# lijrjyan/SDVAR

Measured on AMD Instinct MI355X. Metric: images/s (+ mean accepted tokens/step), VAR-d16 256^2 B=8, d12 draft + d16 verify, per GPU, higher is better.
Workload: dtype f32 (GEMM operands split into 2 fp16 planes to 2^-22, 3 fp16 MFMA products, fp32 accumulate); 1 GPU; BASELINE.json P1: VAR-d16 256^2 B=8/GPU, d12 draft + d16 verify, gamma=2, cfg=1.5 top_k=900 top_p=0.96, acceptance=natural, incl. VQVAE decode (overlapped with the next batch on a 2nd stream); verifier one round behind the draft once gamma = 1; parallelism=1 independent batch shards

## Files before the change

### sdvar_amd/csrc/api.hip

```cpp
#include <math.h>
#include <stdarg.h>
#include <string.h>

#include <vector>

#include "../../include/sdvar_hip.h"
#include "common.h"
#include <string>

namespace sdvar {

int gemm_f32_nt(const float* X, int ldx, const float* W, const float* bias, float* out, int ldo, int M, int N, int K, int epi,
                const float* res, int ldres, const float* gate, int rows_per_gate, int gate_stride, hipStream_t stream);
struct PendingSplitK { const float* ws; const float* bias; const float* gate; int split, rows_per_gate, gate_stride; };
int ln_modulate(float* x, const float* scale, const float* shift, float* out, uint16_t* outp, size_t ops, int rows, int C, int rows_per_img, int mod_stride, const PendingSplitK* pend, int pfmt, hipStream_t stream);
float* splitk_workspace(size_t* floats);
float* set_splitk_workspace(float* p);
size_t splitk_workspace_floats();
int qk_norm_append(const float* qkv, const float* scale_mul, float* q_out, void* k_cache, void* v_cache, int kv_f16, int R, int l, int H, int Lmax, int pos0, const PendingSplitK* pend, int v_only, hipStream_t stream);
int gemm_f16x2_qkv(const uint16_t* X, size_t xps, const uint16_t* W, size_t wps, const float* wsi, const float* bias, float* out, int ldo, int M, int N, int K,
                   const float* scale_mul, float* q_out, void* k_cache, void* v_cache, int l, int H, int Lp, int pos0, int kv_fmt, int* defer, int* fused, hipStream_t stream);
bool gemm_f16x2_rowblk_ok(int M, int N, int K, int ln, int qkv);
bool gemm_f16x2_rowblk_want(int M, int C, int V, int rows_per_img);
int gemm_f16x2_rowblk(const float* x, int ldx, const float* scale, const float* shift, int rows_per_img, int mod_stride, const uint16_t* X, size_t xps,
// ... 9 lines not shown
int build_lvl_pos(const float* lvl_embed, const float* pos, const int* stage_of_tok, float* out, int L, int C, hipStream_t stream);
int embed_next(const float* nxt, const float* Ww, const float* bw, const float* lvl_pos, float* x, int B, int l, int C, int t0, int ltot, int tok_off, int pair, hipStream_t stream);
int xent_stats(const float* logits, const long long* targets, int B, int L, int V, int tail, float* nll_out, long long* argmax_out, double* sums, int accumulate,
               hipStream_t stream);
int attention_f32(const float* q, const void* kc, const void* vc, int kv_f16, float* out, uint16_t* outp, size_t ops, int pfmt, int R, int H, int l, int Lmax, int Ktot, int n_chunk, const int* qbeg, const int* vis, hipStream_t stream);
int gemm_bf16x3_nt(const uint16_t* X, size_t xps, const uint16_t* W, size_t wps, const float* bias, float* out, int ldo, uint16_t* outp, size_t ops,
                   int M, int N, int K, int epi, const float* res, int ldres, const float* gate, int rows_per_gate, int gate_stride, int* defer, hipStream_t stream);
int attention_masked(const float* q, const void* kc, const void* vc, int fmt, const float* bias, float* out, uint16_t* outp, size_t ops, int pfmt, int R, int H, int l,
                     int Lmax, int Ktot, hipStream_t stream);
int split_planes(const float* x, uint16_t* planes, int rows, int cols, size_t plane_stride, hipStream_t stream);
int gemm_f16x2_nt(const uint16_t* X, size_t xps, const uint16_t* W, size_t wps, const float* wsi, const float* bias, float* out, int ldo, uint16_t* outp, size_t ops,
                  int M, int N, int K, int epi, const float* res, int ldres, const float* gate, int rows_per_gate, int gate_stride, int* defer, hipStream_t stream);
int split_planes_f16(const float* x, uint16_t* planes, int rows, int cols, size_t plane_stride, const float* scale, hipStream_t stream);
int weight_scale_f16(const float* w, size_t n, float* sc, hipStream_t stream);
void debug_set_gemm_cfg_h(int bm, int split);
void debug_set_gemm_cfg_p(int bm, int split);
void debug_set_gemm_stamps(unsigned long long* p);
void debug_set_qkv_fuse(int on);
void debug_set_h4_var(int v);
void debug_set_h2_stages(int v);
void debug_set_small_pp(int v);
void debug_set_attn_pp_sched(int v);
void debug_set_conv_pp(int v);
void debug_get_gemm_cfg_h(int* out);
int planes_guard(const uint16_t* h_plane, size_t n, unsigned long long* cnt, hipStream_t stream);
int cfg_sample(const float* logits, int B, int l, int V, float one_plus_t, float t, int top_k, int use_top_p, float top_p_thr, const float* q, uint64_t seed,
               uint32_t draw, uint32_t image_offset, long long* ids, int ids_stride, float* dbg_masked, hipStream_t stream);
int noise_fill(float* q, int B, int l, int V, uint64_t seed, uint32_t draw, uint32_t image_offset, hipStream_t stream);
int verify_accept(const float* logits, int B, int lsum, int V, int n_chunk, const int* qbeg, const float* one_plus_t, const float* t, const long long* draft_ids,
                  int ids_stride, double thr, int mode, int top_k, float kl_thr, const float* draft_logits, const long long* dl_off, int* counts,
                  long long* argmax_out, unsigned char* match_out, long long* corrected_out, hipStream_t stream);
int cfg_combine(const float* logits, int B, int lsum, int V, int n_chunk, const int* qbeg, const float* one_plus_t, const float* t, float* out, hipStream_t stream);
int gumbel_mix(const float* masked, int B, int l, int V, float scale, float tau, const float* e, uint64_t seed, uint32_t draw, uint32_t image_offset,
               const float* codebook, int Cv, float* h, hipStream_t stream);
void debug_set_gemm_cfg(int bm, int split);
int quant_code_norms(const float* codebook, float* e2, int V, int Cv, hipStream_t stream);
int quant_nearest(const float* z, int N, int P, const float* codebook, const float* e2, int V, int Cv, long long* ids, int ids_stride, hipStream_t stream);
int quant_encode_stage(float* f_rest, float* f_hat, float* z, float* up_scratch, const float* codebook, const float* e2, const float* Wdn_si, const float* Wup_si,
                       const float* phi_w, const float* phi_b, long long* ids, int ids_stride, int B, int pn, int HW, int V, int Cv, int last, hipStream_t stream);
int quant_next(const long long* ids, int ids_stride, const float* hvec, const float* codebook, const float* Wup, const float* phi_w, const float* phi_b, const float* Wdn,
               float* up_scratch, const float* f_in, float* f_hat, float* nxt, int B, int pn, int pn_next, int HW, int Cv, int last, hipStream_t stream);

enum { EPI_BIAS = 0, EPI_BIAS_GELU = 1, EPI_GATED_RES = 2 };

static thread_local char g_err[1024] = "";
void set_error(const char* fmt, ...) {
// ... 786 lines not shown
    return SDVAR_OK;
}

int sdvar_debug_set_qkv_fuse(int32_t on) { debug_set_qkv_fuse(on); return SDVAR_OK; }
int sdvar_debug_set_rowblk(int32_t on) { debug_set_rowblk(on); return SDVAR_OK; }
int sdvar_op_gemm_rowblk(const float* x, int32_t ldx, const float* scale, const float* shift, int32_t rows_per_img, int32_t mod_stride, const uint16_t* Xp, uint64_t x_plane_stride,
                         const uint16_t* Wp, uint64_t w_plane_stride, const float* w_scale, const float* bias, float* out, int32_t ldo, uint16_t* out_planes, uint64_t out_plane_stride,
                         int32_t M, int32_t N, int32_t K, int32_t epi, const float* res, int32_t ldres, const float* gate, int32_t rows_per_gate, int32_t gate_stride,
                         const float* scale_mul, float* q_out, void* k_cache, void* v_cache, int32_t l, int32_t H, int32_t Lp, int32_t pos0, int32_t kv_fmt, void* stream) {
    SDVAR_CHECK_ARG(gemm_f16x2_rowblk_ok(M, N, K, x != nullptr, q_out != nullptr), "op_gemm_rowblk: M=%d N=%d K=%d outside the row-block kernel's range (M <= 80; K <= 1024 with a LayerNorm operand, <= 4096 with planes) or the kernel is switched off", M, N, K);
    ProfScope ps(9, 2.0 * M * N * K, 4.0 * ((double)M * K + (double)N * K + (double)M * N), (hipStream_t)stream);
    return gemm_f16x2_rowblk(x, ldx, scale, shift, rows_per_img, mod_stride, Xp, (size_t)x_plane_stride, Wp, (size_t)w_plane_stride, w_scale ? w_scale + 1 : nullptr, bias, out, ldo, out_planes,
                             (size_t)out_plane_stride, M, N, K, epi, res, ldres, gate, rows_per_gate, gate_stride, scale_mul, q_out, k_cache, v_cache, l, H, Lp, pos0, kv_fmt, (hipStream_t)stream);
}

int sdvar_debug_set_variant(const char* name, int32_t value) {
    SDVAR_CHECK_ARG(name, "debug_set_variant: null name");
    const std::string n(name);
    if (n == "gemm_h4_var") { SDVAR_CHECK_ARG(value <= 3, "gemm_h4_var %d", value); debug_set_h4_var(value); }
    else if (n == "gemm_h2_stages") { SDVAR_CHECK_ARG(value < 0 || value == 2 || value == 3 || value == 4 || value == 5 || value == 6, "gemm_h2_stages %d", value); debug_set_h2_stages(value); }
    else if (n == "gemm_small_pp") { SDVAR_CHECK_ARG(value <= 2, "gemm_small_pp %d", value); debug_set_small_pp(value); }
    else if (n == "attn_pp_sched") { SDVAR_CHECK_ARG(value <= 3, "attn_pp_sched %d", value); debug_set_attn_pp_sched(value); }
    else if (n == "conv_pp") { SDVAR_CHECK_ARG(value <= 2, "conv_pp %d", value); debug_set_conv_pp(value); }
    else { set_error("debug_set_variant: unknown variant '%s'", name); return SDVAR_ERR_ARG; }
    return SDVAR_OK;
}

int sdvar_debug_get_gemm_cfg(int32_t* out4) {
    SDVAR_CHECK_ARG(out4, "debug_get_gemm_cfg: null");
    int v[4]; debug_get_gemm_cfg_h(v);
    for (int i = 0; i < 4; ++i) out4[i] = v[i];
    return SDVAR_OK;
}

int sdvar_debug_set_f16x2_guard(int32_t on) {
    if (on && !g_guard_cnt) {
        SDVAR_HIP(hipMalloc((void**)&g_guard_cnt, 4 * sizeof(unsigned long long)));
        SDVAR_HIP(hipMemset(g_guard_cnt, 0, 4 * sizeof(unsigned long long)));
    }
    g_guard_on = on != 0;
    return SDVAR_OK;
}

int sdvar_debug_get_f16x2_guard(uint64_t* out4, int32_t reset) {
    SDVAR_CHECK_ARG(out4, "debug_get_f16x2_guard: null");
    for (int i = 0; i < 4; ++i) out4[i] = 0;
// ... 35 lines not shown
```

### sdvar_amd/csrc/conv.hip

```cpp
#include <stdlib.h>

#include "common.h"

#ifdef SDVAR_TIMING_EXPERIMENTS
#define SDVAR_CDBG(a, bit) ((a).dbg & (bit))
#else
#define SDVAR_CDBG(a, bit) 0
#endif

namespace sdvar {
static int g_conv_pp_override = -1;
void debug_set_conv_pp(int v) { g_conv_pp_override = v; }


typedef __bf16 bf16x8 __attribute__((ext_vector_type(8)));
typedef _Float16 f16x8 __attribute__((ext_vector_type(8)));
typedef __attribute__((address_space(3))) void* lds_ptr_t;
typedef const __attribute__((address_space(1))) void* glb_ptr_t;

enum { CEPI_BIAS = 0, CEPI_BIAS_RES = 1, CEPI_PARTIAL = 2 };
constexpr int CBM = 256, CBN = 160;
constexpr int CSTAGE = 3 * (CBM + CBN) * 32;
constexpr int CSTAGE_H = 2 * (CBM + CBN) * 32;

struct ConvArgs {
    const uint16_t* X; const uint16_t* W;
    size_t xps, wps;
    size_t x_rows;
    int x_row0;
    const float* wsi;
    const float* bias; const float* res; float* out;
    int M, N, cb, taps, ih, iw, ldo, split, k_per_split;
    double* gn_part; int cpg;
    int up_phase;
    size_t w_phase_stride;
    int dbg;
};

template <int EPI>
__device__ __forceinline__ void conv_epilogue(const ConvArgs& a, f32x16 (&acc)[5], float wsi, int m0, int n0, int tm, int ks, int phase, int wave, int li, int lh,
                                              int tid, uint16_t* csm) {
    float rv[5][16];
    if (EPI == CEPI_BIAS_RES) {
#pragma unroll
        for (int j = 0; j < 5; ++j) {
            const int n = n0 + j * 32 + li;
#pragma unroll
            for (int r = 0; r < 16; ++r) {
                const int m = m0 + wave * 32 + (r & 3) + 8 * (r >> 2) + 4 * lh;
                rv[j][r] = (n < a.N && m < a.M) ? a.res[(size_t)m * a.ldo + n] : 0.f;
            }
        }
    }
#pragma unroll
    for (int j = 0; j < 5; ++j) {
        const int n = n0 + j * 32 + li;
        if (n >= a.N) continue;
        const float bv = (EPI != CEPI_PARTIAL && a.bias) ? a.bias[n] : 0.f;
        float* outp = (EPI == CEPI_PARTIAL) ? a.out + (size_t)ks * a.M * a.ldo : a.out;
#pragma unroll
// ... 30 lines not shown
        }
        __syncthreads();
        const int gl = tid, col0 = gl * a.cpg;
        if (col0 < CBN && n0 + col0 < a.N) {
            double a1 = 0.0, a2 = 0.0;
            for (int w = 0; w < 8; ++w)
                for (int c = 0; c < a.cpg; ++c) { a1 += (double)red[w * 160 + col0 + c]; a2 += (double)red[1280 + w * 160 + col0 + c]; }
            double* o = a.gn_part + ((size_t)(a.up_phase >= 0 ? 4 * tm + phase : tm) * 32 + (n0 + col0) / a.cpg) * 2;
            o[0] = a1; o[1] = a2;
        }
    }
}

typedef float cf32x4 __attribute__((ext_vector_type(4)));
__device__ __forceinline__ float dpp_row_sum16(float v) {
    v += __builtin_bit_cast(float, __builtin_amdgcn_update_dpp(0, __builtin_bit_cast(int, v), 0x111, 0xF, 0xF, true));
    v += __builtin_bit_cast(float, __builtin_amdgcn_update_dpp(0, __builtin_bit_cast(int, v), 0x112, 0xF, 0xF, true));
    v += __builtin_bit_cast(float, __builtin_amdgcn_update_dpp(0, __builtin_bit_cast(int, v), 0x114, 0xF, 0xF, true));
    v += __builtin_bit_cast(float, __builtin_amdgcn_update_dpp(0, __builtin_bit_cast(int, v), 0x118, 0xF, 0xF, true));
    return v;
}
template <int EPI>
__device__ __forceinline__ void conv_epilogue16(const ConvArgs& a, cf32x4 (&acc)[2][10], float wsi, int m0, int n0, int tm, int ks, int phase, int wave, int l15, int lq,
                                                int tid, uint16_t* csm) {
    int mrow[2]; size_t orow[2];
#pragma unroll
    for (int mt = 0; mt < 2; ++mt) {
        const int m = m0 + wave * 32 + 16 * mt + l15;
        mrow[mt] = m; orow[mt] = (size_t)m;
        if (EPI != CEPI_PARTIAL && a.up_phase >= 0 && m < a.M) {
            const int hw = a.ih * a.iw, b = m / hw, rem = m - b * hw, y = rem / a.iw, x = rem - y * a.iw;
            orow[mt] = ((size_t)(b * 2 * a.ih + 2 * y + (phase >> 1)) * (2 * a.iw) + 2 * x + (phase & 1));
        }
    }
    cf32x4 rv[2][10];
    if (EPI == CEPI_BIAS_RES) {
#pragma unroll
        for (int mt = 0; mt < 2; ++mt)
#pragma unroll
            for (int nt = 0; nt < 10; ++nt) {
                const int n = n0 + 16 * nt + 4 * lq;
                rv[mt][nt] = (n < a.N && mrow[mt] < a.M) ? *reinterpret_cast<const cf32x4*>(a.res + (size_t)mrow[mt] * a.ldo + n) : cf32x4{0.f, 0.f, 0.f, 0.f};
            }
    }
    float* outp = (EPI == CEPI_PARTIAL) ? a.out + (size_t)ks * a.M * a.ldo : a.out;
#pragma unroll
    for (int nt = 0; nt < 10; ++nt) {
        const int n = n0 + 16 * nt + 4 * lq;
        if (n >= a.N) continue;
        const cf32x4 bv = (EPI != CEPI_PARTIAL && a.bias) ? *reinterpret_cast<const cf32x4*>(a.bias + n) : cf32x4{0.f, 0.f, 0.f, 0.f};
#pragma unroll
        for (int mt = 0; mt < 2; ++mt) {
            if (mrow[mt] >= a.M) continue;
            cf32x4 v;
#pragma unroll
            for (int e = 0; e < 4; ++e) { v[e] = acc[mt][nt][e] * wsi + bv[e]; if (EPI == CEPI_BIAS_RES) v[e] += rv[mt][nt][e]; }
            if (!SDVAR_CDBG(a, 4)) *reinterpret_cast<cf32x4*>(outp + orow[mt] * a.ldo + n) = v;
            acc[mt][nt] = v;
        }
    }
    if (EPI != CEPI_PARTIAL && a.gn_part && !SDVAR_CDBG(a, 2)) {
        float* red = reinterpret_cast<float*>(csm);
        __syncthreads();
#pragma unroll
        for (int nt = 0; nt < 10; ++nt)
#pragma unroll
            for (int e = 0; e < 4; ++e) {
                const bool in = n0 + 16 * nt + 4 * lq < a.N;
                const float x0 = in ? acc[0][nt][e] : 0.f, x1 = in ? acc[1][nt][e] : 0.f;
                const float s1 = dpp_row_sum16(x0 + x1), s2 = dpp_row_sum16(x0 * x0 + x1 * x1);
                if (l15 == 15) { red[wave * 160 + 16 * nt + 4 * lq + e] = s1; red[1280 + wave * 160 + 16 * nt + 4 * lq + e] = s2; }
            }
        __syncthreads();
        const int gl = tid, col0 = gl * a.cpg;
        if (col0 < CBN && n0 + col0 < a.N) {
            double a1 = 0.0, a2 = 0.0;
            for (int w = 0; w < 8; ++w)
                for (int c = 0; c < a.cpg; ++c) { a1 += (double)red[w * 160 + col0 + c]; a2 += (double)red[1280 + w * 160 + col0 + c]; }
            double* o = a.gn_part + ((size_t)(a.up_phase >= 0 ? 4 * tm + phase : tm) * 32 + (n0 + col0) / a.cpg) * 2;
            o[0] = a1; o[1] = a2;
        }
    }
}

template <int EPI>
// ... 94 lines not shown
                __builtin_amdgcn_sched_barrier(0);
                if (s == 0 && j == 0) {
                    SDVAR_LDS_RD(fb[1][1][4], ab1, 18432);
                    SDVAR_RD_B(1, ab1, 0, 0);
                }
                if (pf) {
                    const int grp = 5 * s + j;
                    issue_one(nst, grp);
                    if (grp >= 8) issue_one(nst, grp + 2);
                }
                __builtin_amdgcn_sched_barrier(0);
            }
        }
#undef SDVAR_RD_B
#undef SDVAR_LDS_RD
    }

    conv_epilogue<EPI>(a, acc, 1.0f, m0, n0, tm, ks, phase, wave, li, lh, tid, csm);
}

template <int EPI, int PP>
__global__ __launch_bounds__(512, 2) void conv_f16x2_kernel(ConvArgs a) {
    extern __shared__ __attribute__((aligned(16))) uint16_t csm[];
    const int tiles_m = (a.M + CBM - 1) / CBM, tiles_n = (a.N + CBN - 1) / CBN, ntile = tiles_m * tiles_n;
    const int ks = blockIdx.x / ntile;
    const int lid = xcd_remap(blockIdx.x - ks * ntile, ntile);
    const int tm = lid / tiles_n, tn = lid - tm * tiles_n;
    const int m0 = tm * CBM, n0 = tn * CBN;

    const int tid = threadIdx.x, lane = tid & 63, wave = tid >> 6;
    const int li = lane & 31, lh = lane >> 5;
    const int phase = a.up_phase >= 0 ? (int)blockIdx.y : 0;
    const uint16_t* Wp = a.W + (size_t)phase * a.w_phase_stride;

    const int r16 = lane >> 2;
    const int xr0 = 32 * wave + r16, xr1 = xr0 + 16, wr0 = 16 * wave + r16, wr1 = 128 + wr0;
    const int cx0 = (lane & 3) ^ ((xr0 >> 2) & 3), cx1 = (lane & 3) ^ ((xr1 >> 2) & 3), cw0 = (lane & 3) ^ ((wr0 >> 2) & 3), cw1 = (lane & 3) ^ ((wr1 >> 2) & 3);
    const int nkt = a.taps * a.cb;
    const int kt0 = ks * a.k_per_split;
    const int nk = min(nkt - kt0, a.k_per_split);
    const int w2 = a.iw + 2;
    auto prow = [&](int m) {
        const int hw = a.ih * a.iw, b = m / hw, rem = m - b * hw, y = rem / a.iw, x = rem - y * a.iw;
        return (size_t)(b * (a.ih + 2) + y + 1) * w2 + x + 1;
    };
    const int swave = __builtin_amdgcn_readfirstlane(wave);
    const uint32_t lx0 = (uint32_t)((a.x_row0 + prow(min(m0 + xr0, a.M - 1))) * 32 + 8 * cx0) * 2u;
    const uint32_t lx1 = (uint32_t)((a.x_row0 + prow(min(m0 + xr1, a.M - 1))) * 32 + 8 * cx1) * 2u;
    const uint32_t lw0 = (uint32_t)(min(n0 + wr0, a.N - 1) * 32 + 8 * cw0) * 2u, lw1 = (uint32_t)(min(n0 + wr1, a.N - 1) * 32 + 8 * cw1) * 2u;
    const bool two_w = swave < 2;
    const char* ux = nullptr; const char* uw = nullptr;
    const int tw = (a.taps == 9) ? 3 : 2;
    int sc = kt0 % a.cb, stap = kt0 / a.cb, sty = stap / tw, stx = stap - sty * tw, skb = kt0;
    auto set_next = [&]() {
        const int shift = (a.taps == 9) ? (sty - 1) * w2 + (stx - 1) : (a.taps == 4) ? (sty - 1 + (phase >> 1)) * w2 + (stx - 1 + (phase & 1)) : 0;
        ux = reinterpret_cast<const char*>(a.X) + ((long long)sc * (long long)a.x_rows + shift) * 64;
        uw = reinterpret_cast<const char*>(Wp) + (size_t)skb * a.N * 64;
        ++skb;
        if (++sc == a.cb) { sc = 0; if (++stx == tw) { stx = 0; ++sty; } }
    };
    auto issue_one = [&](uint16_t* st, int q) {
        if (q < 6) {
            const int p = q / 3, kind = q % 3;
            if (kind == 0) SDVAR_DMA16(lx0, ux + p * a.xps * 2, SDVAR_LDS_ADDR(st + p * 8192 + swave * 1024));
            else if (kind == 1) SDVAR_DMA16(lx1, ux + p * a.xps * 2, SDVAR_LDS_ADDR(st + p * 8192 + swave * 1024 + 512));
            else SDVAR_DMA16(lw0, uw + p * a.wps * 2, SDVAR_LDS_ADDR(st + 2 * 8192 + p * 5120 + swave * 512));
        } else if (two_w) {
            const int p = q - 6;
            SDVAR_DMA16(lw1, uw + p * a.wps * 2, SDVAR_LDS_ADDR(st + 2 * 8192 + p * 5120 + 4096 + swave * 512));
        }
    };

    f32x16 acc[5];
#pragma unroll
    for (int j = 0; j < 5; ++j)
#pragma unroll
        for (int r = 0; r < 16; ++r) acc[j][r] = 0.f;

    const int sw = (li >> 2) & 3;
    const int offa = (wave * 32 + li) * 32, offb = 2 * 8192 + li * 32;
    const int ch0 = 8 * ((0 + lh) ^ sw), ch1 = 8 * ((2 + lh) ^ sw);

    set_next();
#pragma unroll
    for (int q = 0; q < 8; ++q) issue_one(csm, q);
    if (nk > 1) {
        set_next();
#pragma unroll
        for (int q = 0; q < 8; ++q) issue_one(csm + CSTAGE_H, q);
    }
    if constexpr (PP == 2) {
        const int late = __builtin_amdgcn_readfirstlane(wave >> 2);
        const int l15 = lane & 15, lq = lane >> 4;
        auto wait_next = [&](int t) {
            if (t + 2 < nk) { if (two_w) asm volatile("s_waitcnt vmcnt(8)" ::: "memory"); else asm volatile("s_waitcnt vmcnt(6)" ::: "memory"); }
            else asm volatile("s_waitcnt vmcnt(0)" ::: "memory");
        };
#define SDVAR_C_SLOT() do { __builtin_amdgcn_sched_barrier(0); __builtin_amdgcn_s_barrier(); __builtin_amdgcn_sched_barrier(0); } while (0)
#define SDVAR_LDS_RD(dst, addr, off) asm volatile("ds_read_b128 %0, %1 offset:" #off : "=v"(dst) : "v"(addr) : "memory")
#define SDVAR_C_MFMA16(J0)                                                                                      \
        _Pragma("unroll") for (int j = 0; j < 5; ++j)                                                           \
            _Pragma("unroll") for (int i = 0; i < 2; ++i) {                                                     \
                acc16[i][(J0) + j] = __builtin_amdgcn_mfma_f32_16x16x32_f16(fw[j][0], fx[i][1], acc16[i][(J0) + j], 0, 0, 0);   \
                acc16[i][(J0) + j] = __builtin_amdgcn_mfma_f32_16x16x32_f16(fw[j][1], fx[i][0], acc16[i][(J0) + j], 0, 0, 0);   \
                acc16[i][(J0) + j] = __builtin_amdgcn_mfma_f32_16x16x32_f16(fw[j][0], fx[i][0], acc16[i][(J0) + j], 0, 0, 0);   \
            }
        cf32x4 acc16[2][10];
#pragma unroll
        for (int i = 0; i < 2; ++i)
#pragma unroll
            for (int j = 0; j < 10; ++j)
#pragma unroll
                for (int r = 0; r < 4; ++r) acc16[i][j][r] = 0.f;
        const uint32_t fro = (uint32_t)(l15 * 64 + 16 * (lq ^ ((l15 >> 2) & 3)));
        const uint32_t fxo = (uint32_t)(wave * 32 * 64) + fro, fwo = 32768u + fro;
        wait_next(-1);
        SDVAR_C_SLOT();
        if (late) SDVAR_C_SLOT();
        f16x8 fx[2][2], fw[5][2];
#pragma unroll 1
        for (int t = 0; t < nk; ++t) {
            const bool pf = t + 2 < nk;
            uint16_t* nst = csm + ((t + 2) % 3) * CSTAGE_H;
            const uint32_t sb = (uint32_t)(uintptr_t)(lds_ptr_t)(csm + (t % 3) * CSTAGE_H);
            const uint32_t xa = sb + fxo, wa = sb + fwo;
            SDVAR_LDS_RD(fx[0][0], xa, 0); SDVAR_LDS_RD(fx[0][1], xa, 16384); SDVAR_LDS_RD(fx[1][0], xa, 1024); SDVAR_LDS_RD(fx[1][1], xa, 17408);
            SDVAR_LDS_RD(fw[0][0], wa, 0);    SDVAR_LDS_RD(fw[0][1], wa, 10240); SDVAR_LDS_RD(fw[1][0], wa, 1024); SDVAR_LDS_RD(fw[1][1], wa, 11264);
            SDVAR_LDS_RD(fw[2][0], wa, 2048); SDVAR_LDS_RD(fw[2][1], wa, 12288); SDVAR_LDS_RD(fw[3][0], wa, 3072); SDVAR_LDS_RD(fw[3][1], wa, 13312);
            SDVAR_LDS_RD(fw[4][0], wa, 4096); SDVAR_LDS_RD(fw[4][1], wa, 14336);
            if (pf) {
                set_next();
#pragma unroll
                for (int q = 0; q < 4; ++q) issue_one(nst, q);
            }
            asm volatile("s_waitcnt lgkmcnt(0)" ::: "memory");
            SDVAR_C_SLOT();
            SDVAR_C_MFMA16(0);
            SDVAR_C_SLOT();
            SDVAR_LDS_RD(fw[0][0], wa, 5120); SDVAR_LDS_RD(fw[0][1], wa, 15360); SDVAR_LDS_RD(fw[1][0], wa, 6144); SDVAR_LDS_RD(fw[1][1], wa, 16384);
            SDVAR_LDS_RD(fw[2][0], wa, 7168); SDVAR_LDS_RD(fw[2][1], wa, 17408); SDVAR_LDS_RD(fw[3][0], wa, 8192); SDVAR_LDS_RD(fw[3][1], wa, 18432);
            SDVAR_LDS_RD(fw[4][0], wa, 9216); SDVAR_LDS_RD(fw[4][1], wa, 19456);
            if (pf) {
#pragma unroll
                for (int q = 4; q < 8; ++q) issue_one(nst, q);
            }
            if (late) wait_next(t);
            asm volatile("s_waitcnt lgkmcnt(0)" ::: "memory");
            SDVAR_C_SLOT();
            SDVAR_C_MFMA16(5);
            if (!late) wait_next(t);
            SDVAR_C_SLOT();
        }
        if (!late) SDVAR_C_SLOT();
#undef SDVAR_C_MFMA16
#undef SDVAR_LDS_RD
#undef SDVAR_C_SLOT
        if (SDVAR_CDBG(a, 1)) return;
        conv_epilogue16<EPI>(a, acc16, a.wsi ? *a.wsi : 1.0f, m0, n0, tm, ks, phase, wave, l15, lq, tid, csm);
        return;
    } else
    if (PP) {
        const int late = __builtin_amdgcn_readfirstlane(wave >> 2);
        auto wait_next = [&](int t) {
            if (t + 2 < nk) { if (two_w) asm volatile("s_waitcnt vmcnt(8)" ::: "memory"); else asm volatile("s_waitcnt vmcnt(6)" ::: "memory"); }
            else asm volatile("s_waitcnt vmcnt(0)" ::: "memory");
        };
#define SDVAR_C_SLOT() do { __builtin_amdgcn_sched_barrier(0); __builtin_amdgcn_s_barrier(); __builtin_amdgcn_sched_barrier(0); } while (0)
#define SDVAR_LDS_RD(dst, addr, off) asm volatile("ds_read_b128 %0, %1 offset:" #off : "=v"(dst) : "v"(addr) : "memory")
#define SDVAR_RD_B(ab, p, pb) SDVAR_LDS_RD(fb[p][0], ab, pb); SDVAR_LDS_RD(fb[p][1], ab, pb + 2048); SDVAR_LDS_RD(fb[p][2], ab, pb + 4096); \
                              SDVAR_LDS_RD(fb[p][3], ab, pb + 6144); SDVAR_LDS_RD(fb[p][4], ab, pb + 8192)
#define SDVAR_C_MFMA()                                                                                  \
        _Pragma("unroll") for (int j = 0; j < 5; ++j) {                                                 \
            acc[j] = __builtin_amdgcn_mfma_f32_32x32x16_f16(fa[1], fb[0][j], acc[j], 0, 0, 0);          \
            acc[j] = __builtin_amdgcn_mfma_f32_32x32x16_f16(fa[0], fb[1][j], acc[j], 0, 0, 0);          \
            acc[j] = __builtin_amdgcn_mfma_f32_32x32x16_f16(fa[0], fb[0][j], acc[j], 0, 0, 0);          \
        }
        wait_next(-1);
        SDVAR_C_SLOT();
        if (late) SDVAR_C_SLOT();
        f16x8 fa[2], fb[2][5];
#pragma unroll 1
// ... 52 lines not shown
#undef SDVAR_RD_B
#undef SDVAR_LDS_RD
#pragma unroll
        for (int s = 0; s < 2; ++s) {
            if (s == 0) asm volatile("s_waitcnt lgkmcnt(12)" ::: "memory");
            else asm volatile("s_waitcnt lgkmcnt(0)" ::: "memory");
            __builtin_amdgcn_sched_barrier(0);
#pragma unroll
            for (int j = 0; j < 5; ++j) {
                acc[j] = __builtin_amdgcn_mfma_f32_32x32x16_f16(fa[s][1], fb[s][0][j], acc[j], 0, 0, 0);
                acc[j] = __builtin_amdgcn_mfma_f32_32x32x16_f16(fa[s][0], fb[s][1][j], acc[j], 0, 0, 0);
                acc[j] = __builtin_amdgcn_mfma_f32_32x32x16_f16(fa[s][0], fb[s][0][j], acc[j], 0, 0, 0);
                __builtin_amdgcn_sched_barrier(0);
                if (pf) {
                    const int grp = 5 * s + j;
                    if (grp < 8) issue_one(nst, grp);
                }
                __builtin_amdgcn_sched_barrier(0);
            }
        }
    }
    if (SDVAR_CDBG(a, 1)) return;
    conv_epilogue<EPI>(a, acc, a.wsi ? *a.wsi : 1.0f, m0, n0, tm, ks, phase, wave, li, lh, tid, csm);
}

__global__ __launch_bounds__(256) void conv_reduce_kernel(const float* __restrict__ ws, int split, const float* __restrict__ bias, const float* res,
                                                          float* out, int M, int N) {
    const int nv = N >> 2;
    const size_t total = (size_t)M * nv, slab = (size_t)M * N;
    for (size_t i = (size_t)blockIdx.x * blockDim.x + threadIdx.x; i < total; i += (size_t)gridDim.x * blockDim.x) {
        const int n = (int)(i % nv) * 4;
        f32x4 acc = *reinterpret_cast<const f32x4*>(ws + 4 * i);
        for (int s = 1; s < split; ++s) {
            const f32x4 p = *reinterpret_cast<const f32x4*>(ws + s * slab + 4 * i);
            acc[0] += p[0]; acc[1] += p[1]; acc[2] += p[2]; acc[3] += p[3];
        }
        if (bias) { const f32x4 b = *reinterpret_cast<const f32x4*>(bias + n); acc[0] += b[0]; acc[1] += b[1]; acc[2] += b[2]; acc[3] += b[3]; }
        if (res) { const f32x4 r = *reinterpret_cast<const f32x4*>(res + 4 * i); acc[0] += r[0]; acc[1] += r[1]; acc[2] += r[2]; acc[3] += r[3]; }
        *reinterpret_cast<f32x4*>(out + 4 * i) = acc;
    }
}

__global__ __launch_bounds__(256) void conv_weight_planes_kernel(const float* __restrict__ w, uint16_t* __restrict__ p, int Cout, int Cin, int taps, size_t ps, int pfmt,
                                                                 const float* scale) {
    const int K = taps * Cin;
    const size_t total = (size_t)Cout * K;
// ... 38 lines not shown
}

int upconv_weights(const float* w, float* weff, int Cout, int Cin, hipStream_t stream) {
    hipLaunchKernelGGL(upconv_weight_kernel, dim3(1024), dim3(256), 0, stream, w, weff, Cout, Cin);
    SDVAR_LAUNCH_CHECK();
    return SDVAR_OK;
}

static int conv_choose_split(int M, int N, int nkt, size_t ws_floats, double kstep_cycles) {
    const long tiles = (long)((M + CBM - 1) / CBM) * ((N + CBN - 1) / CBN);
    double best = 1e30; int bs = 1;
    for (int split = 1; split <= 16 && split <= nkt / 2; ++split) {
        if (split > 1 && ((size_t)split * M * N > ws_floats || N % 4)) break;
        const int kps = (nkt + split - 1) / split;
        if ((nkt + kps - 1) / kps != split) continue;
        const long rounds = (tiles * split + 255) / 256;
        double cyc = (double)rounds * (kps * kstep_cycles + 3000.0);
        if (split > 1) cyc += 4000.0 + (double)(split + 2) * M * N * 4.0 / 4000.0;
        if (cyc < best) { best = cyc; bs = split; }
    }
    return bs;
}

int conv_planes(const uint16_t* X, size_t xps, size_t x_rows, int x_row0, const uint16_t* W, size_t wps, int pfmt, const float* wsi, const float* bias, const float* res,
                float* out, int B, int H, int Wd, int N, int Cin, int taps, float* ws, size_t ws_floats, int force_split, double* gn_part, int* gn_done, int up_phase,
                size_t w_phase_stride, hipStream_t stream) {
    if (gn_done) *gn_done = 0;
    const int M = B * H * Wd, w2 = Wd + 2;
    const size_t Mp = (size_t)B * (H + 2) * w2;
    SDVAR_CHECK_ARG(X && W && out, "conv: null operand");
    SDVAR_CHECK_ARG(M > 0 && N > 0 && Cin > 0 && Cin % 32 == 0 && (taps == 1 || taps == 9 || (taps == 4 && up_phase >= 0)) && (taps == 4 || up_phase < 0), "conv: M=%d N=%d Cin=%d taps=%d", M, N, Cin, taps);
    SDVAR_CHECK_ARG(B > 0 && H > 0 && Wd > 0 && x_row0 >= w2 + 1, "conv: guard rows %d < row pitch %d + 1", x_row0, w2);
    SDVAR_CHECK_ARG(x_rows >= (size_t)x_row0 + Mp + w2 + 1, "conv: plane rows %zu too few", x_rows);
    SDVAR_CHECK_ARG(((uintptr_t)X % 16) == 0 && ((uintptr_t)W % 16) == 0 && xps % 8 == 0 && wps % 8 == 0, "conv: planes must be 16-byte aligned");
    SDVAR_CHECK_ARG(pfmt == PLANES_BF16X3 || pfmt == PLANES_F16X2, "conv: plane format %d", pfmt);
    const bool F16 = pfmt == PLANES_F16X2;
    ConvArgs a{X, W, xps, wps, x_rows, x_row0, F16 ? wsi : nullptr, bias, res, out, M, N, Cin / 32, taps, H, Wd, N, 1, taps * (Cin / 32), nullptr, 1, up_phase, w_phase_stride, 0};
#ifdef SDVAR_TIMING_EXPERIMENTS
    static const int conv_dbg = getenv("SDVAR_CONV_DBG") ? atoi(getenv("SDVAR_CONV_DBG")) : 0;
    a.dbg = conv_dbg;
#else
    a.dbg = 0;
#endif
    const int nkt = taps * (Cin / 32);
    const int tiles = ((M + CBM - 1) / CBM) * ((N + CBN - 1) / CBN);
    int split = up_phase >= 0 ? 1 : force_split > 0 ? force_split : conv_choose_split(M, N, nkt, ws ? ws_floats : 0, F16 ? 1200.0 : 2100.0);
    if (split > nkt) split = nkt;
    if (split > 1) {
        SDVAR_CHECK_ARG(ws && (size_t)split * M * N <= ws_floats && N % 4 == 0, "conv: split-K workspace too small");
        const int kps = (nkt + split - 1) / split;
        split = (nkt + kps - 1) / kps;
        a.k_per_split = kps; a.split = split;
    }
    const size_t lds = F16 ? 3 * (size_t)CSTAGE_H * sizeof(uint16_t) : 2 * (size_t)CSTAGE * sizeof(uint16_t);
    const char* pp_s = getenv("SDVAR_CONV_PP");
    const int pp_env = g_conv_pp_override >= 0 ? g_conv_pp_override : (pp_s ? atoi(pp_s) : 2);
    const int pp = (pp_env == 2 && N % 4 != 0) ? 1 : pp_env;
    static LdsOptIn opt_in, opt_in_h;
    if (F16) SDVAR_LDS_OPT_IN(opt_in_h, lds, (const void*)conv_f16x2_kernel<CEPI_BIAS, 0>, (const void*)conv_f16x2_kernel<CEPI_BIAS_RES, 0>, (const void*)conv_f16x2_kernel<CEPI_PARTIAL, 0>,
                              (const void*)conv_f16x2_kernel<CEPI_BIAS, 1>, (const void*)conv_f16x2_kernel<CEPI_BIAS_RES, 1>, (const void*)conv_f16x2_kernel<CEPI_PARTIAL, 1>,
                              (const void*)conv_f16x2_kernel<CEPI_BIAS, 2>, (const void*)conv_f16x2_kernel<CEPI_BIAS_RES, 2>, (const void*)conv_f16x2_kernel<CEPI_PARTIAL, 2>);
    else SDVAR_LDS_OPT_IN(opt_in, lds, (const void*)conv_bf16x3_kernel<CEPI_BIAS>, (const void*)conv_bf16x3_kernel<CEPI_BIAS_RES>, (const void*)conv_bf16x3_kernel<CEPI_PARTIAL>);
    if (split > 1) {
        ConvArgs p = a;
        p.out = ws;
        if (F16 && pp == 2) hipLaunchKernelGGL((conv_f16x2_kernel<CEPI_PARTIAL, 2>), dim3(tiles * split), dim3(512), lds, stream, p);
        else if (F16 && pp) hipLaunchKernelGGL((conv_f16x2_kernel<CEPI_PARTIAL, 1>), dim3(tiles * split), dim3(512), lds, stream, p);
        else if (F16) hipLaunchKernelGGL((conv_f16x2_kernel<CEPI_PARTIAL, 0>), dim3(tiles * split), dim3(512), lds, stream, p);
        else hipLaunchKernelGGL((conv_bf16x3_kernel<CEPI_PARTIAL>), dim3(tiles * split), dim3(512), lds, stream, p);
        SDVAR_LAUNCH_CHECK();
        const size_t total = (size_t)M * (N / 4);
        const int rgrid = (int)((total + 255) / 256 < 4096 ? (total + 255) / 256 : 4096);
        hipLaunchKernelGGL(conv_reduce_kernel, dim3(rgrid), dim3(256), 0, stream, ws, split, bias, res, out, M, N);
        SDVAR_LAUNCH_CHECK();
        return SDVAR_OK;
    }
    if (gn_part && N % 32 == 0 && CBN % (N / 32) == 0 && (H * Wd) % CBM == 0) { a.gn_part = gn_part; a.cpg = N / 32; if (gn_done) *gn_done = 1; }
    if (F16) {
        if (res && pp == 2) hipLaunchKernelGGL((conv_f16x2_kernel<CEPI_BIAS_RES, 2>), dim3(tiles), dim3(512), lds, stream, a);
        else if (res && pp) hipLaunchKernelGGL((conv_f16x2_kernel<CEPI_BIAS_RES, 1>), dim3(tiles), dim3(512), lds, stream, a);
        else if (res) hipLaunchKernelGGL((conv_f16x2_kernel<CEPI_BIAS_RES, 0>), dim3(tiles), dim3(512), lds, stream, a);
        else if (pp == 2) hipLaunchKernelGGL((conv_f16x2_kernel<CEPI_BIAS, 2>), dim3(tiles, up_phase >= 0 ? 4 : 1), dim3(512), lds, stream, a);
        else if (pp) hipLaunchKernelGGL((conv_f16x2_kernel<CEPI_BIAS, 1>), dim3(tiles, up_phase >= 0 ? 4 : 1), dim3(512), lds, stream, a);
        else hipLaunchKernelGGL((conv_f16x2_kernel<CEPI_BIAS, 0>), dim3(tiles, up_phase >= 0 ? 4 : 1), dim3(512), lds, stream, a);
    } else if (res) hipLaunchKernelGGL((conv_bf16x3_kernel<CEPI_BIAS_RES>), dim3(tiles), dim3(512), lds, stream, a);
    else hipLaunchKernelGGL((conv_bf16x3_kernel<CEPI_BIAS>), dim3(tiles, up_phase >= 0 ? 4 : 1), dim3(512), lds, stream, a);
    SDVAR_LAUNCH_CHECK();
    return SDVAR_OK;
}

}
```

Measured before the change: 182.9 images/s.

## Process multiple conv tiles per workgroup, overlapping next tile's prologue with epilogue

The PP=2 f16x2 conv kernel becomes persistent over a group of tiles (tpw, default 2 when the grid exceeds 256 workgroups). While the current tile's epilogue runs, the next tile's first loads are already issued. The epilogue now uses the third LDS stage as scratch so it does not clash with the in-flight prefetch. This aims to hide load latency between tiles and cut workgroup launch overhead in the VQVAE decode convs. The cost is fewer workgroups, which may leave CUs idle, plus optional timing-stamp instrumentation.

```diff
diff --git a/sdvar_amd/csrc/api.hip b/sdvar_amd/csrc/api.hip
--- a/sdvar_amd/csrc/api.hip
+++ b/sdvar_amd/csrc/api.hip
@@ -55,6 +55,7 @@
 void debug_set_small_pp(int v);
 void debug_set_attn_pp_sched(int v);
 void debug_set_conv_pp(int v);
+void debug_set_conv_tiles(int v);
 void debug_get_gemm_cfg_h(int* out);
 int planes_guard(const uint16_t* h_plane, size_t n, unsigned long long* cnt, hipStream_t stream);
 int cfg_sample(const float* logits, int B, int l, int V, float one_plus_t, float t, int top_k, int use_top_p, float top_p_thr, const float* q, uint64_t seed,
@@ -887,6 +888,7 @@
     else if (n == "gemm_small_pp") { SDVAR_CHECK_ARG(value <= 2, "gemm_small_pp %d", value); debug_set_small_pp(value); }
     else if (n == "attn_pp_sched") { SDVAR_CHECK_ARG(value <= 3, "attn_pp_sched %d", value); debug_set_attn_pp_sched(value); }
     else if (n == "conv_pp") { SDVAR_CHECK_ARG(value <= 2, "conv_pp %d", value); debug_set_conv_pp(value); }
+    else if (n == "conv_tiles") { SDVAR_CHECK_ARG(value <= 64, "conv_tiles %d", value); debug_set_conv_tiles(value); }
     else { set_error("debug_set_variant: unknown variant '%s'", name); return SDVAR_ERR_ARG; }
     return SDVAR_OK;
 }
diff --git a/sdvar_amd/csrc/conv.hip b/sdvar_amd/csrc/conv.hip
--- a/sdvar_amd/csrc/conv.hip
+++ b/sdvar_amd/csrc/conv.hip
@@ -11,6 +11,11 @@
 namespace sdvar {
 static int g_conv_pp_override = -1;
 void debug_set_conv_pp(int v) { g_conv_pp_override = v; }
+static int g_conv_tiles_override = -1;
+void debug_set_conv_tiles(int v) { g_conv_tiles_override = v; }
+#ifdef SDVAR_CONV_STAMPS
+unsigned long long* debug_get_gemm_stamps();
+#endif
 
 
 typedef __bf16 bf16x8 __attribute__((ext_vector_type(8)));
@@ -35,7 +40,15 @@
     int up_phase;
     size_t w_phase_stride;
     int dbg;
+    int tpw;
+#ifdef SDVAR_CONV_STAMPS
+    unsigned long long* stamps;
+    int epi;
+#endif
 };
+#ifdef SDVAR_CONV_STAMPS
+constexpr size_t CSTAMP_SLOT = 8 + 16384, CSTAMP_SLOTS = 128;
+#endif
 
 template <int EPI>
 __device__ __forceinline__ void conv_epilogue(const ConvArgs& a, f32x16 (&acc)[5], float wsi, int m0, int n0, int tm, int ks, int phase, int wave, int li, int lh,
@@ -112,7 +125,7 @@
 }
 template <int EPI>
 __device__ __forceinline__ void conv_epilogue16(const ConvArgs& a, cf32x4 (&acc)[2][10], float wsi, int m0, int n0, int tm, int ks, int phase, int wave, int l15, int lq,
-                                                int tid, uint16_t* csm) {
+                                                int tid, uint16_t* scratch) {
     int mrow[2]; size_t orow[2];
 #pragma unroll
     for (int mt = 0; mt < 2; ++mt) {
@@ -150,7 +163,7 @@
         }
     }
     if (EPI != CEPI_PARTIAL && a.gn_part && !SDVAR_CDBG(a, 2)) {
-        float* red = reinterpret_cast<float*>(csm);
+        float* red = reinterpret_cast<float*>(scratch);
         __syncthreads();
 #pragma unroll
         for (int nt = 0; nt < 10; ++nt)
@@ -291,11 +304,17 @@
 template <int EPI, int PP>
 __global__ __launch_bounds__(512, 2) void conv_f16x2_kernel(ConvArgs a) {
     extern __shared__ __attribute__((aligned(16))) uint16_t csm[];
+#ifdef SDVAR_CONV_STAMPS
+    unsigned long long csr[4] = {0, 0, 0, 0}, csc[4] = {0, 0, 0, 0};
+#define SDVAR_CONV_STAMP(k) do { csr[k] = __builtin_amdgcn_s_memrealtime(); csc[k] = __builtin_amdgcn_s_memtime(); } while (0)
+    SDVAR_CONV_STAMP(0);
+#else
+#define SDVAR_CONV_STAMP(k) do { } while (0)
+#endif
     const int tiles_m = (a.M + CBM - 1) / CBM, tiles_n = (a.N + CBN - 1) / CBN, ntile = tiles_m * tiles_n;
-    const int ks = blockIdx.x / ntile;
-    const int lid = xcd_remap(blockIdx.x - ks * ntile, ntile);
-    const int tm = lid / tiles_n, tn = lid - tm * tiles_n;
-    const int m0 = tm * CBM, n0 = tn * CBN;
+    const int ngrp = (ntile + a.tpw - 1) / a.tpw;
+    const int ks = blockIdx.x / ngrp;
+    const int lid0 = xcd_remap(blockIdx.x - ks * ngrp, ngrp) * a.tpw;
 
     const int tid = threadIdx.x, lane = tid & 63, wave = tid >> 6;
     const int li = lane & 31, lh = lane >> 5;
@@ -314,13 +333,19 @@
         return (size_t)(b * (a.ih + 2) + y + 1) * w2 + x + 1;
     };
     const int swave = __builtin_amdgcn_readfirstlane(wave);
-    const uint32_t lx0 = (uint32_t)((a.x_row0 + prow(min(m0 + xr0, a.M - 1))) * 32 + 8 * cx0) * 2u;
-    const uint32_t lx1 = (uint32_t)((a.x_row0 + prow(min(m0 + xr1, a.M - 1))) * 32 + 8 * cx1) * 2u;
-    const uint32_t lw0 = (uint32_t)(min(n0 + wr0, a.N - 1) * 32 + 8 * cw0) * 2u, lw1 = (uint32_t)(min(n0 + wr1, a.N - 1) * 32 + 8 * cw1) * 2u;
     const bool two_w = swave < 2;
+    const int tw = (a.taps == 9) ? 3 : 2;
+    int tm, tn, m0, n0, sc, sty, stx, skb;
+    uint32_t lx0, lx1, lw0, lw1;
+    auto set_tile = [&](int l) {
+        tm = l / tiles_n; tn = l - tm * tiles_n; m0 = tm * CBM; n0 = tn * CBN;
+        lx0 = (uint32_t)((a.x_row0 + prow(min(m0 + xr0, a.M - 1))) * 32 + 8 * cx0) * 2u;
+        lx1 = (uint32_t)((a.x_row0 + prow(min(m0 + xr1, a.M - 1))) * 32 + 8 * cx1) * 2u;
+        lw0 = (uint32_t)(min(n0 + wr0, a.N - 1) * 32 + 8 * cw0) * 2u; lw1 = (uint32_t)(min(n0 + wr1, a.N - 1) * 32 + 8 * cw1) * 2u;
+        const int stap = kt0 / a.cb;
+        sc = kt0 % a.cb; sty = stap / tw; stx = stap - sty * tw; skb = kt0;
+    };
     const char* ux = nullptr; const char* uw = nullptr;
-    const int tw = (a.taps == 9) ? 3 : 2;
-    int sc = kt0 % a.cb, stap = kt0 / a.cb, sty = stap / tw, stx = stap - sty * tw, skb = kt0;
     auto set_next = [&]() {
         const int shift = (a.taps == 9) ? (sty - 1) * w2 + (stx - 1) : (a.taps == 4) ? (sty - 1 + (phase >> 1)) * w2 + (stx - 1 + (phase & 1)) : 0;
         ux = reinterpret_cast<const char*>(a.X) + ((long long)sc * (long long)a.x_rows + shift) * 64;
@@ -339,6 +364,16 @@
             SDVAR_DMA16(lw1, uw + p * a.wps * 2, SDVAR_LDS_ADDR(st + 2 * 8192 + p * 5120 + 4096 + swave * 512));
         }
     };
+    auto prologue = [&]() {
+        set_next();
+#pragma unroll
+        for (int q = 0; q < 8; ++q) issue_one(csm, q);
+        if (nk > 1) {
+            set_next();
+#pragma unroll
+            for (int q = 0; q < 8; ++q) issue_one(csm + CSTAGE_H, q);
+        }
+    };
 
     f32x16 acc[5];
 #pragma unroll
@@ -350,14 +385,8 @@
     const int offa = (wave * 32 + li) * 32, offb = 2 * 8192 + li * 32;
     const int ch0 = 8 * ((0 + lh) ^ sw), ch1 = 8 * ((2 + lh) ^ sw);
 
-    set_next();
-#pragma unroll
-    for (int q = 0; q < 8; ++q) issue_one(csm, q);
-    if (nk > 1) {
-        set_next();
-#pragma unroll
-        for (int q = 0; q < 8; ++q) issue_one(csm + CSTAGE_H, q);
-    }
+    set_tile(lid0);
+    prologue();
     if constexpr (PP == 2) {
         const int late = __builtin_amdgcn_readfirstlane(wave >> 2);
         const int l15 = lane & 15, lq = lane >> 4;
@@ -374,58 +403,85 @@
                 acc16[i][(J0) + j] = __builtin_amdgcn_mfma_f32_16x16x32_f16(fw[j][1], fx[i][0], acc16[i][(J0) + j], 0, 0, 0);   \
                 acc16[i][(J0) + j] = __builtin_amdgcn_mfma_f32_16x16x32_f16(fw[j][0], fx[i][0], acc16[i][(J0) + j], 0, 0, 0);   \
             }
-        cf32x4 acc16[2][10];
-#pragma unroll
-        for (int i = 0; i < 2; ++i)
-#pragma unroll
-            for (int j = 0; j < 10; ++j)
-#pragma unroll
-                for (int r = 0; r < 4; ++r) acc16[i][j][r] = 0.f;
         const uint32_t fro = (uint32_t)(l15 * 64 + 16 * (lq ^ ((l15 >> 2) & 3)));
         const uint32_t fxo = (uint32_t)(wave * 32 * 64) + fro, fwo = 32768u + fro;
-        wait_next(-1);
-        SDVAR_C_SLOT();
-        if (late) SDVAR_C_SLOT();
+        const float wsi = a.wsi ? *a.wsi : 1.0f;
         f16x8 fx[2][2], fw[5][2];
 #pragma unroll 1
-        for (int t = 0; t < nk; ++t) {
-            const bool pf = t + 2 < nk;
-            uint16_t* nst = csm + ((t + 2) % 3) * CSTAGE_H;
-            const uint32_t sb = (uint32_t)(uintptr_t)(lds_ptr_t)(csm + (t % 3) * CSTAGE_H);
-            const uint32_t xa = sb + fxo, wa = sb + fwo;
-            SDVAR_LDS_RD(fx[0][0], xa, 0); SDVAR_LDS_RD(fx[0][1], xa, 16384); SDVAR_LDS_RD(fx[1][0], xa, 1024); SDVAR_LDS_RD(fx[1][1], xa, 17408);
-            SDVAR_LDS_RD(fw[0][0], wa, 0);    SDVAR_LDS_RD(fw[0][1], wa, 10240); SDVAR_LDS_RD(fw[1][0], wa, 1024); SDVAR_LDS_RD(fw[1][1], wa, 11264);
-            SDVAR_LDS_RD(fw[2][0], wa, 2048); SDVAR_LDS_RD(fw[2][1], wa, 12288); SDVAR_LDS_RD(fw[3][0], wa, 3072); SDVAR_LDS_RD(fw[3][1], wa, 13312);
-            SDVAR_LDS_RD(fw[4][0], wa, 4096); SDVAR_LDS_RD(fw[4][1], wa, 14336);
-            if (pf) {
-                set_next();
-#pragma unroll
-                for (int q = 0; q < 4; ++q) issue_one(nst, q);
-            }
-            asm volatile("s_waitcnt lgkmcnt(0)" ::: "memory");
+        for (int it = 0;;) {
+            cf32x4 acc16[2][10];
+#pragma unroll
+            for (int i = 0; i < 2; ++i)
+#pragma unroll
+                for (int j = 0; j < 10; ++j)
+#pragma unroll
+                    for (int r = 0; r < 4; ++r) acc16[i][j][r] = 0.f;
+            wait_next(-1);
             SDVAR_C_SLOT();
-            SDVAR_C_MFMA16(0);
-            SDVAR_C_SLOT();
-            SDVAR_LDS_RD(fw[0][0], wa, 5120); SDVAR_LDS_RD(fw[0][1], wa, 15360); SDVAR_LDS_RD(fw[1][0], wa, 6144); SDVAR_LDS_RD(fw[1][1], wa, 16384);
-            SDVAR_LDS_RD(fw[2][0], wa, 7168); SDVAR_LDS_RD(fw[2][1], wa, 17408); SDVAR_LDS_RD(fw[3][0], wa, 8192); SDVAR_LDS_RD(fw[3][1], wa, 18432);
-            SDVAR_LDS_RD(fw[4][0], wa, 9216); SDVAR_LDS_RD(fw[4][1], wa, 19456);
-            if (pf) {
-#pragma unroll
-                for (int q = 4; q < 8; ++q) issue_one(nst, q);
-            }
-            if (late) wait_next(t);
-            asm volatile("s_waitcnt lgkmcnt(0)" ::: "memory");
-            SDVAR_C_SLOT();
-            SDVAR_C_MFMA16(5);
-            if (!late) wait_next(t);
-            SDVAR_C_SLOT();
-        }
-        if (!late) SDVAR_C_SLOT();
+            SDVAR_CONV_STAMP(1);
+            if (late) SDVAR_C_SLOT();
+#pragma unroll 1
+            for (int t = 0; t < nk; ++t) {
+                const bool pf = t + 2 < nk;
+                uint16_t* nst = csm + ((t + 2) % 3) * CSTAGE_H;
+                const uint32_t sb = (uint32_t)(uintptr_t)(lds_ptr_t)(csm + (t % 3) * CSTAGE_H);
+                const uint32_t xa = sb + fxo, wa = sb + fwo;
+                SDVAR_LDS_RD(fx[0][0], xa, 0); SDVAR_LDS_RD(fx[0][1], xa, 16384); SDVAR_LDS_RD(fx[1][0], xa, 1024); SDVAR_LDS_RD(fx[1][1], xa, 17408);
+                SDVAR_LDS_RD(fw[0][0], wa, 0);    SDVAR_LDS_RD(fw[0][1], wa, 10240); SDVAR_LDS_RD(fw[1][0], wa, 1024); SDVAR_LDS_RD(fw[1][1], wa, 11264);
+                SDVAR_LDS_RD(fw[2][0], wa, 2048); SDVAR_LDS_RD(fw[2][1], wa, 12288); SDVAR_LDS_RD(fw[3][0], wa, 3072); SDVAR_LDS_RD(fw[3][1], wa, 13312);
+                SDVAR_LDS_RD(fw[4][0], wa, 4096); SDVAR_LDS_RD(fw[4][1], wa, 14336);
+                if (pf) {
+                    set_next();
+#pragma unroll
+                    for (int q = 0; q < 4; ++q) issue_one(nst, q);
+                }
+                asm volatile("s_waitcnt lgkmcnt(0)" ::: "memory");
+                SDVAR_C_SLOT();
+                SDVAR_C_MFMA16(0);
+                SDVAR_C_SLOT();
+                SDVAR_LDS_RD(fw[0][0], wa, 5120); SDVAR_LDS_RD(fw[0][1], wa, 15360); SDVAR_LDS_RD(fw[1][0], wa, 6144); SDVAR_LDS_RD(fw[1][1], wa, 16384);
+                SDVAR_LDS_RD(fw[2][0], wa, 7168); SDVAR_LDS_RD(fw[2][1], wa, 17408); SDVAR_LDS_RD(fw[3][0], wa, 8192); SDVAR_LDS_RD(fw[3][1], wa, 18432);
+                SDVAR_LDS_RD(fw[4][0], wa, 9216); SDVAR_LDS_RD(fw[4][1], wa, 19456);
+                if (pf) {
+#pragma unroll
+                    for (int q = 4; q < 8; ++q) issue_one(nst, q);
+                }
+                if (late) wait_next(t);
+                asm volatile("s_waitcnt lgkmcnt(0)" ::: "memory");
+                SDVAR_C_SLOT();
+                SDVAR_C_MFMA16(5);
+                if (!late) wait_next(t);
+                SDVAR_C_SLOT();
+            }
+            if (!late) SDVAR_C_SLOT();
+            SDVAR_CONV_STAMP(2);
+            const int cm0 = m0, cn0 = n0, ctm = tm;
+#ifdef SDVAR_CONV_STAMPS
+            const int clid = lid0 + it;
+#endif
+            const bool more = ++it < a.tpw && lid0 + it < ntile;
+            if (more) { set_tile(lid0 + it); prologue(); }
+            if (!SDVAR_CDBG(a, 1)) conv_epilogue16<EPI>(a, acc16, wsi, cm0, cn0, ctm, ks, phase, wave, l15, lq, tid, csm + 2 * CSTAGE_H);
+#ifdef SDVAR_CONV_STAMPS
+            SDVAR_CONV_STAMP(3);
+            if (a.stamps && tid == 0) {
+                const size_t o = 8 + (((size_t)blockIdx.y * a.split + ks) * ntile + clid) * 8;
+                if (o + 8 <= CSTAMP_SLOT)
+#pragma unroll
+                    for (int k = 0; k < 4; ++k) { a.stamps[o + k] = csr[k]; a.stamps[o + 4 + k] = csc[k]; }
+                if (blockIdx.x == 0 && blockIdx.y == 0 && clid == lid0) {
+                    const long long h[8] = {a.M, a.N, a.taps, a.up_phase, a.epi, a.tpw, a.split, nk};
+#pragma unroll
+                    for (int k = 0; k < 8; ++k) a.stamps[k] = (unsigned long long)h[k];
+                }
+            }
+            SDVAR_CONV_STAMP(0);
+#endif
+            if (!more) break;
+        }
 #undef SDVAR_C_MFMA16
 #undef SDVAR_LDS_RD
 #undef SDVAR_C_SLOT
-        if (SDVAR_CDBG(a, 1)) return;
-        conv_epilogue16<EPI>(a, acc16, a.wsi ? *a.wsi : 1.0f, m0, n0, tm, ks, phase, wave, l15, lq, tid, csm);
         return;
     } else
     if (PP) {
@@ -524,6 +580,7 @@
     }
     if (SDVAR_CDBG(a, 1)) return;
     conv_epilogue<EPI>(a, acc, a.wsi ? *a.wsi : 1.0f, m0, n0, tm, ks, phase, wave, li, lh, tid, csm);
+#undef SDVAR_CONV_STAMP
 }
 
 __global__ __launch_bounds__(256) void conv_reduce_kernel(const float* __restrict__ ws, int split, const float* __restrict__ bias, const float* res,
@@ -608,6 +665,14 @@
     return bs;
 }
 
+static int conv_tiles_per_wg(int wgs) {
+    constexpr int DEFAULT_ROUNDS = 1, DEFAULT_T = 2;
+    const char* s = getenv("SDVAR_CONV_TILES");
+    const int v = g_conv_tiles_override > 0 ? g_conv_tiles_override : (s && atoi(s) > 0) ? atoi(s) : 0;
+    if (v > 0) return v;
+    return wgs > DEFAULT_ROUNDS * 256 ? DEFAULT_T : 1;
+}
+
 int conv_planes(const uint16_t* X, size_t xps, size_t x_rows, int x_row0, const uint16_t* W, size_t wps, int pfmt, const float* wsi, const float* bias, const float* res,
                 float* out, int B, int H, int Wd, int N, int Cin, int taps, float* ws, size_t ws_floats, int force_split, double* gn_part, int* gn_done, int up_phase,
                 size_t w_phase_stride, hipStream_t stream) {
@@ -621,7 +686,7 @@
     SDVAR_CHECK_ARG(((uintptr_t)X % 16) == 0 && ((uintptr_t)W % 16) == 0 && xps % 8 == 0 && wps % 8 == 0, "conv: planes must be 16-byte aligned");
     SDVAR_CHECK_ARG(pfmt == PLANES_BF16X3 || pfmt == PLANES_F16X2, "conv: plane format %d", pfmt);
     const bool F16 = pfmt == PLANES_F16X2;
-    ConvArgs a{X, W, xps, wps, x_rows, x_row0, F16 ? wsi : nullptr, bias, res, out, M, N, Cin / 32, taps, H, Wd, N, 1, taps * (Cin / 32), nullptr, 1, up_phase, w_phase_stride, 0};
+    ConvArgs a{X, W, xps, wps, x_rows, x_row0, F16 ? wsi : nullptr, bias, res, out, M, N, Cin / 32, taps, H, Wd, N, 1, taps * (Cin / 32), nullptr, 1, up_phase, w_phase_stride, 0, 1};
 #ifdef SDVAR_TIMING_EXPERIMENTS
     static const int conv_dbg = getenv("SDVAR_CONV_DBG") ? atoi(getenv("SDVAR_CONV_DBG")) : 0;
     a.dbg = conv_dbg;
@@ -647,6 +712,11 @@
                               (const void*)conv_f16x2_kernel<CEPI_BIAS, 1>, (const void*)conv_f16x2_kernel<CEPI_BIAS_RES, 1>, (const void*)conv_f16x2_kernel<CEPI_PARTIAL, 1>,
                               (const void*)conv_f16x2_kernel<CEPI_BIAS, 2>, (const void*)conv_f16x2_kernel<CEPI_BIAS_RES, 2>, (const void*)conv_f16x2_kernel<CEPI_PARTIAL, 2>);
     else SDVAR_LDS_OPT_IN(opt_in, lds, (const void*)conv_bf16x3_kernel<CEPI_BIAS>, (const void*)conv_bf16x3_kernel<CEPI_BIAS_RES>, (const void*)conv_bf16x3_kernel<CEPI_PARTIAL>);
+#ifdef SDVAR_CONV_STAMPS
+    static unsigned stamp_seq = 0;
+    a.stamps = nullptr; a.epi = split > 1 ? CEPI_PARTIAL : res ? CEPI_BIAS_RES : CEPI_BIAS;
+    if (debug_get_gemm_stamps() && F16 && pp == 2) a.stamps = debug_get_gemm_stamps() + (size_t)(stamp_seq++ % CSTAMP_SLOTS) * CSTAMP_SLOT;
+#endif
     if (split > 1) {
         ConvArgs p = a;
         p.out = ws;
@@ -663,10 +733,12 @@
     }
     if (gn_part && N % 32 == 0 && CBN % (N / 32) == 0 && (H * Wd) % CBM == 0) { a.gn_part = gn_part; a.cpg = N / 32; if (gn_done) *gn_done = 1; }
     if (F16) {
-        if (res && pp == 2) hipLaunchKernelGGL((conv_f16x2_kernel<CEPI_BIAS_RES, 2>), dim3(tiles), dim3(512), lds, stream, a);
+        if (pp == 2) a.tpw = conv_tiles_per_wg(tiles * (up_phase >= 0 ? 4 : 1));
+        const int grid = (tiles + a.tpw - 1) / a.tpw;
+        if (res && pp == 2) hipLaunchKernelGGL((conv_f16x2_kernel<CEPI_BIAS_RES, 2>), dim3(grid), dim3(512), lds, stream, a);
         else if (res && pp) hipLaunchKernelGGL((conv_f16x2_kernel<CEPI_BIAS_RES, 1>), dim3(tiles), dim3(512), lds, stream, a);
         else if (res) hipLaunchKernelGGL((conv_f16x2_kernel<CEPI_BIAS_RES, 0>), dim3(tiles), dim3(512), lds, stream, a);
-        else if (pp == 2) hipLaunchKernelGGL((conv_f16x2_kernel<CEPI_BIAS, 2>), dim3(tiles, up_phase >= 0 ? 4 : 1), dim3(512), lds, stream, a);
+        else if (pp == 2) hipLaunchKernelGGL((conv_f16x2_kernel<CEPI_BIAS, 2>), dim3(grid, up_phase >= 0 ? 4 : 1), dim3(512), lds, stream, a);
         else if (pp) hipLaunchKernelGGL((conv_f16x2_kernel<CEPI_BIAS, 1>), dim3(tiles, up_phase >= 0 ? 4 : 1), dim3(512), lds, stream, a);
         else hipLaunchKernelGGL((conv_f16x2_kernel<CEPI_BIAS, 0>), dim3(tiles, up_phase >= 0 ? 4 : 1), dim3(512), lds, stream, a);
     } else if (res) hipLaunchKernelGGL((conv_bf16x3_kernel<CEPI_BIAS_RES>), dim3(tiles), dim3(512), lds, stream, a);
```

Measured after the change: 180.5 images/s, median of 2. 1.3% lower.
